# arturxe2/T-DEED

Hardware: AMD Instinct MI355X
Metric: clips/sec (L=100, 224^2, bf16) forward, per-frame logits (higher is better)
Workload: dtype bf16; 1 GPU; rny002_b8: rny002_gsf + ed_sgp_mixer n_layers=2 ks=7, L=100, 224x224, batch 8/GPU, inference forward, random-init weights; clips_per_gpu=8, parallelism=dp1 (clip-sharded, no collective), hip_graph=True, batches_in_flight=3, sub_batches_per_batch=1, dist_backend=none, dist_ranks=1, self_launched=False

## Files before the change

t-deed_amd/csrc/bneck.hip:

```cpp
#include "common.h"
#include "se_excite.h"

struct BneckP {
  const bf16_t* x; const bf16_t* G; int Fp;
  const bf16x8* w1f; const float* s1; const float* h1;
  const bf16x8* w2f; const float* s2; const float* h2;
  SeP se;
  const bf16x8* w3f; const float* s3; const float* h3;
  bf16_t* out; bf16_t* out2; int n2;
  int N, h, w, C;
  int w2_tap_major;
  long long* dbg;
  struct Gs {
    const bf16_t* x; int ldx;
    const float* gate; const float* ysum; const float* xsum;
    const float* cw1; const float* cb1; const float* cw2; const float* cb2;
    int T_len, F;
  } gs;
  struct Qt {
    const bf16x8* wqf;
    const float* bn;
    float* Q;
    int F;
  } qt;
// ... 154 lines not shown
#pragma unroll
      for (int b = 0; b < NLD; ++b) {
        const int i = i0 + b * BNK_THR;
        if (i < total) {
          int px, ck;
          dcpr.divmod(i, px, ck);
          ck += ck0;
          TD_LDS_CHECK(px * RS + ck * 16, 16, FPW * hw * RS);
          *reinterpret_cast<u32x4*>(At + px * RS + ck * 16) = v[b];
        }
      }
    };
    x_issue(tid);
    TD_ISSUE_FENCE();
    if (blend) {
      if (sfs < nfr && sc_ < gF) {
        const int f = f0 + sfs, t = f - dgt.div(f) * gT;
#pragma unroll
        for (int row = 0; row < 10; ++row) {
          const int t2 = t + (row >= 5 ? row - 5 : row) - 2;
          srow(1 + 12 * sfs + row)[sc_] = (t2 >= 0 && t2 < gT) ? sv[row] : 0.f;
        }
      }
      float* cwl = srow(1 + 12 * FPW);
      if (tid >= 256 && tid < 256 + 38) cwl[tid - 256] = cwv;
      __syncthreads();
      {
        const int fs = (FPW > 1 && tid >= p.Fp) ? 1 : 0, c = tid - fs * p.Fp;
        if (fs < nfr && c < p.Fp) {
          const int t = (f0 + fs) - dgt.div(f0 + fs) * gT;
          const int rb = 1 + 12 * fs;
          const float inv_hw = 1.0f / (float)hw;
          float wgt = 0.f;
          if (c < gF) {
            const int g = c >= gFh;
            const int cl = c - g * gFh;
            const float* cw = cwl + 18 * g;
            float a = cwl[36 + g];
#pragma unroll
            for (int dc = -1; dc <= 1; ++dc) {
              const int c2 = cl + dc;
              if (c2 < 0 || c2 >= gFh) continue;
              const int cc = g * gFh + c2;
#pragma unroll
              for (int dt = -1; dt <= 1; ++dt) {
                const int t2 = t + dt;
                if (t2 < 0 || t2 >= gT) continue;
                const float rm = (srow(rb + 5 + dt + 2)[cc] - srow(rb + dt + 2)[cc]) * inv_hw;
                const int r2 = dt + 2 + (g ? -1 : 1);
                const float ysh = srow(rb + r2)[cc] * inv_hw;
                a = fmaf(cw[(dc + 1) * 3 + (dt + 1)], ysh, a);
                a = fmaf(cw[9 + (dc + 1) * 3 + (dt + 1)], rm, a);
              }
            }
            wgt = sigmoidf_(a);
          }
          TD_LDS_CHECK((Bt - smem) + (rb + 11) * RS + c * 4, 4, (Zr - smem));
          srow(rb + 10)[c] = wgt;
          srow(rb + 11)[c] = 1.0f - wgt;
        }
      }
      __syncthreads();
      const IDiv dnpc(npc8);
#pragma unroll
      for (int j = 0; j < 3; ++j) {
        const int i = tid + j * BNK_THR;
        if (i < npix * npc8) {
          int px, ck;
          dnpc.divmod(i, px, ck);
          const int fs = (FPW > 1 && px >= hw) ? 1 : 0;
          const int t = (f0 + fs) - dgt.div(f0 + fs) * gT;
          const bool has_next = t < gT - 1, has_prev = t > 0;
          const float* fwl = srow(1 + 12 * fs + 10) + ck * 8;
          const float* oml = srow(1 + 12 * fs + 11) + ck * 8;
          const f32x4 w0 = *reinterpret_cast<const f32x4*>(fwl), w1 = *reinterpret_cast<const f32x4*>(fwl + 4);
          const f32x4 m0 = *reinterpret_cast<const f32x4*>(oml), m1 = *reinterpret_cast<const f32x4*>(oml + 4);
          const float gn_ = has_next ? bgn[j] : 0.f, gp_ = has_prev ? bgp[j] : 0.f;
          const bool lo_piece = ck * 8 < gFh;
          u32x4 o;
#pragma unroll
          for (int pr = 0; pr < 4; ++pr) {
            const int ci = ck * 8 + 2 * pr;
            const bool g = ci >= gFh;
            const unsigned xcw = bxc[j][pr], nbw = (g && lo_piece) ? bxp[j][pr] : bxn[j][pr];
            const f32x2 xv = {__builtin_bit_cast(float, xcw << 16), __builtin_bit_cast(float, xcw & 0xffff0000u)};
            const f32x2 nb = {__builtin_bit_cast(float, nbw << 16), __builtin_bit_cast(float, nbw & 0xffff0000u)};
            const float gate = g ? bga[j][1] : bga[j][0], gsh = g ? gp_ : gn_;
            const f32x2 gate2 = {gate, gate}, gsh2 = {gsh, gsh};
            const f32x2 wv = pr < 2 ? (f32x2){w0[2 * pr], w0[2 * pr + 1]} : (f32x2){w1[2 * pr - 4], w1[2 * pr - 3]};
            const f32x2 om = pr < 2 ? (f32x2){m0[2 * pr], m0[2 * pr + 1]} : (f32x2){m1[2 * pr - 4], m1[2 * pr - 3]};
            const f32x2 r = __builtin_elementwise_fma(-gate2, xv, xv);
            const f32x2 ysh = gsh2 * nb;
            const f32x2 t = r * om;
            const f32x2 ov = __builtin_elementwise_fma(ysh, wv, t);
            const bf16x2 ob = {(bf16_t)ov[0], (bf16_t)ov[1]};
            o[pr] = ci < gF ? __builtin_bit_cast(unsigned, ob) : xcw;
          }
          TD_LDS_CHECK(px * RS + ck * 16, 16, FPW * hw * RS);
          *reinterpret_cast<u32x4*>(At + px * RS + ck * 16) = o;
        }
      }
    }
    x_store(tid);
    for (int i0 = tid + BNK_THR * NLD; i0 < total; i0 += BNK_THR * NLD) {
      x_issue(i0);
      TD_ISSUE_FENCE();
      x_store(i0);
    }
    const int padp = (RS - C * 2) >> 4;
    for (int i = tid; i < 2 * FPW * hw * padp; i += BNK_THR) {
      const int r = i / padp, j = i - r * padp;
      *reinterpret_cast<u32x4*>(smem + r * RS + C * 2 + j * 16) = (u32x4){0u, 0u, 0u, 0u};
    }
    for (int i = tid; i < (RS + 64) >> 4; i += BNK_THR) *reinterpret_cast<u32x4*>(Zr + i * 16) = (u32x4){0u, 0u, 0u, 0u};
    if (tid < 4) *reinterpret_cast<u32x4*>(At + npix * RS + tid * 16) = (u32x4){0u, 0u, 0u, 0u};
#pragma unroll
    for (int j = 0; j < NBV; ++j) {
      const int i = tid + j * BNK_THR;
      if (i < 6 * CP) bnv[i] = (i - (i / CP) * CP) < C ? bv[j] : 0.f;
    }
  }
  __syncthreads();
  BN_STAMP(1);

  int prow[NPTM], srowA[NPTM];
#pragma unroll
  for (int pt = 0; pt < NPTM; ++pt) {
    const int px = pt * 16 + pl;
    prow[pt] = (px < npix ? px : 0) * RS;
    srowA[pt] = px < npix ? px * RS : (int)(Tr - At);
  }
  const int dAB = (int)(Bt - At);
  constexpr int HA = (NPTM + 1) / 2;
  auto contract = [&](const bf16x8 (&wc)[KS], const unsigned char* act, f32x4 (&acc)[NPTM]) {
#pragma unroll
    for (int pt = 0; pt < NPTM; ++pt) acc[pt] = (f32x4){0.f, 0.f, 0.f, 0.f};
    bf16x8 a[NPTM];
    const int kq = 16 * q;
#pragma unroll
    for (int pt = 0; pt < HA; ++pt) a[pt] = *reinterpret_cast<const bf16x8*>(act + prow[pt] + kq);
#pragma unroll
    for (int ks = 0; ks < KS; ++ks) {
      const int kb = 64 * ks + kq;
#pragma unroll
      for (int pt = HA; pt < NPTM; ++pt) a[pt] = *reinterpret_cast<const bf16x8*>(act + prow[pt] + kb);
#pragma unroll
      for (int pt = 0; pt < HA; ++pt) acc[pt] = __builtin_amdgcn_mfma_f32_16x16x32_bf16(wc[ks], a[pt], acc[pt], 0, 0, 0);
      __builtin_amdgcn_sched_barrier(0);
      if (ks + 1 < KS) {
#pragma unroll
        for (int pt = 0; pt < HA; ++pt) a[pt] = *reinterpret_cast<const bf16x8*>(act + prow[pt] + kb + 64);
      }
#pragma unroll
      for (int pt = HA; pt < NPTM; ++pt) acc[pt] = __builtin_amdgcn_mfma_f32_16x16x32_bf16(wc[ks], a[pt], acc[pt], 0, 0, 0);
      __builtin_amdgcn_sched_barrier(0);
    }
  };

  auto contract_half = [&](const bf16x8 (&wb)[KS], int ks0, const unsigned char* act, f32x4 (&acc0)[NPTM], f32x4 (&acc1)[NPTM]) {
    bf16x8 a[NPTM];
    const int kq = 16 * q;
#pragma unroll
    for (int pt = 0; pt < HA; ++pt) a[pt] = *reinterpret_cast<const bf16x8*>(act + prow[pt] + 64 * ks0 + kq);
#pragma unroll
    for (int k = 0; k < KH; ++k) {
      const int kb = 64 * (ks0 + k) + kq;
#pragma unroll
      for (int pt = HA; pt < NPTM; ++pt) a[pt] = *reinterpret_cast<const bf16x8*>(act + prow[pt] + kb);
#pragma unroll
      for (int pt = 0; pt < HA; ++pt) {
        acc0[pt] = __builtin_amdgcn_mfma_f32_16x16x32_bf16(wb[k], a[pt], acc0[pt], 0, 0, 0);
        acc1[pt] = __builtin_amdgcn_mfma_f32_16x16x32_bf16(wb[KH + k], a[pt], acc1[pt], 0, 0, 0);
      }
      __builtin_amdgcn_sched_barrier(0);
      if (k + 1 < KH) {
#pragma unroll
        for (int pt = 0; pt < HA; ++pt) a[pt] = *reinterpret_cast<const bf16x8*>(act + prow[pt] + kb + 64);
      }
#pragma unroll
      for (int pt = HA; pt < NPTM; ++pt) {
        acc0[pt] = __builtin_amdgcn_mfma_f32_16x16x32_bf16(wb[k], a[pt], acc0[pt], 0, 0, 0);
        acc1[pt] = __builtin_amdgcn_mfma_f32_16x16x32_bf16(wb[KH + k], a[pt], acc1[pt], 0, 0, 0);
      }
      __builtin_amdgcn_sched_barrier(0);
    }
  };
  auto contract_third = [&](const bf16x8 (&wb)[KS], int ks0, const unsigned char* act, f32x4 (&acc0)[NPTM], f32x4 (&acc1)[NPTM],
                            f32x4 (&acc2)[NPTM]) {
    bf16x8 a[NPTM];
    const int kq = 16 * q;
#pragma unroll
    for (int pt = 0; pt < HA; ++pt) a[pt] = *reinterpret_cast<const bf16x8*>(act + prow[pt] + 64 * ks0 + kq);
#pragma unroll
    for (int k = 0; k < KT; ++k) {
      const int kb = 64 * (ks0 + k) + kq;
#pragma unroll
      for (int pt = HA; pt < NPTM; ++pt) a[pt] = *reinterpret_cast<const bf16x8*>(act + prow[pt] + kb);
#pragma unroll
      for (int pt = 0; pt < HA; ++pt) {
        acc0[pt] = __builtin_amdgcn_mfma_f32_16x16x32_bf16(wb[k], a[pt], acc0[pt], 0, 0, 0);
        acc1[pt] = __builtin_amdgcn_mfma_f32_16x16x32_bf16(wb[KT + k], a[pt], acc1[pt], 0, 0, 0);
        acc2[pt] = __builtin_amdgcn_mfma_f32_16x16x32_bf16(wb[2 * KT + k], a[pt], acc2[pt], 0, 0, 0);
      }
      __builtin_amdgcn_sched_barrier(0);
      if (k + 1 < KT) {
#pragma unroll
        for (int pt = 0; pt < HA; ++pt) a[pt] = *reinterpret_cast<const bf16x8*>(act + prow[pt] + kb + 64);
      }
#pragma unroll
      for (int pt = HA; pt < NPTM; ++pt) {
        acc0[pt] = __builtin_amdgcn_mfma_f32_16x16x32_bf16(wb[k], a[pt], acc0[pt], 0, 0, 0);
        acc1[pt] = __builtin_amdgcn_mfma_f32_16x16x32_bf16(wb[KT + k], a[pt], acc1[pt], 0, 0, 0);
        acc2[pt] = __builtin_amdgcn_mfma_f32_16x16x32_bf16(wb[2 * KT + k], a[pt], acc2[pt], 0, 0, 0);
      }
      __builtin_amdgcn_sched_barrier(0);
    }
  };
  auto epi1 = [&](int T, const f32x4 (&acc)[NPTM]) {
    const int ch0 = T * 16 + 4 * q;
    const f32x4 sc = *reinterpret_cast<const f32x4*>(bnv + ch0), sh = *reinterpret_cast<const f32x4*>(bnv + CP + ch0);
#pragma unroll
    for (int pt = 0; pt < NPTM; ++pt) {
      bf16x4 o;
#pragma unroll
      for (int r = 0; r < 4; ++r) o[r] = (bf16_t)fmaxf(acc[pt][r] * sc[r] + sh[r], 0.f);
      unsigned char* dst = At + srowA[pt];
      TD_LDS_CHECK(((srowA[pt] < dAB ? dst + dAB : dst) + ch0 * 2) - smem, 8, (Tr + RS) - smem);
      *reinterpret_cast<bf16x4*>((srowA[pt] < dAB ? dst + dAB : dst) + ch0 * 2) = o;
    }
  };

  if constexpr (TRIPLE) {
    bf16x8 (&wn)[KS] = wn1;
    f32x4 acc0[NPTM], acc1[NPTM], acc2[NPTM];
#pragma unroll
    for (int pt = 0; pt < NPTM; ++pt) acc0[pt] = acc1[pt] = acc2[pt] = (f32x4){0.f, 0.f, 0.f, 0.f};
    contract_third(wc1, 0, At, acc0, acc1, acc2);
    load_block3(wc1, p.w1f, T3A, T3B, T3C, 2 * KT);
    contract_third(wn, KT, At, acc0, acc1, acc2);
    if (wv < NT) {
#pragma unroll
      for (int ks = 0; ks < 5; ++ks) wf2[ks] = p.w2f[((long)wv * 5 + ks) * 64 + lane];
    }
    contract_third(wc1, 2 * KT, At, acc0, acc1, acc2);
    epi1(T3A, acc0);
    epi1(T3B, acc1);
    if (t3c_ok) epi1(wv + 2 * BNK_NW, acc2);
  } else if constexpr (PAIR) {
    bf16x8 wn[KS];
    if (wv < NT) {
#pragma unroll
      for (int ks = 0; ks < 5; ++ks) wf2[ks] = p.w2f[((long)wv * 5 + ks) * 64 + lane];
    }
    const int TA = wv, TB = wv + BNK_NW, TC = wv + 2 * BNK_NW;
    load_block(wn, p.w1f, TA, TB, KH);
    f32x4 acc0[NPTM], acc1[NPTM];
#pragma unroll
    for (int pt = 0; pt < NPTM; ++pt) acc0[pt] = acc1[pt] = (f32x4){0.f, 0.f, 0.f, 0.f};
    contract_half(wc1, 0, At, acc0, acc1);
    if (TC < NT) {
#pragma unroll
      for (int ks = 0; ks < KS; ++ks) wc1[ks] = p.w1f[((long)TC * KS + ks) * 64 + lane];
    }
    contract_half(wn, KH, At, acc0, acc1);
    epi1(TA, acc0);
    epi1(TB, acc1);
    if (TC < NT) {
      contract(wc1, At, acc0);
      epi1(TC, acc0);
    }
  } else {
    bf16x8 (&wc)[KS] = wc1;
    bf16x8 wn[KS];
    if (wv < NT) {
#pragma unroll
      for (int ks = 0; ks < 5; ++ks) wf2[ks] = p.w2f[((long)wv * 5 + ks) * 64 + lane];
    }
    for (int T = wv; T < NT; T += BNK_NW) {
      if (T + BNK_NW < NT) {
#pragma unroll
        for (int ks = 0; ks < KS; ++ks) wn[ks] = p.w1f[((long)(T + BNK_NW) * KS + ks) * 64 + lane];
      }
      const int ch0 = T * 16 + 4 * q;
      const f32x4 sc = *reinterpret_cast<const f32x4*>(bnv + ch0), sh = *reinterpret_cast<const f32x4*>(bnv + CP + ch0);
      f32x4 acc[NPTM];
      contract(wc, At, acc);
#pragma unroll
      for (int pt = 0; pt < NPTM; ++pt) {
        bf16x4 o;
#pragma unroll
        for (int r = 0; r < 4; ++r) o[r] = (bf16_t)fmaxf(acc[pt][r] * sc[r] + sh[r], 0.f);
        unsigned char* dst = At + srowA[pt];
        TD_LDS_CHECK(((srowA[pt] < dAB ? dst + dAB : dst) + ch0 * 2) - smem, 8, (Tr + RS) - smem);
        *reinterpret_cast<bf16x4*>((srowA[pt] < dAB ? dst + dAB : dst) + ch0 * 2) = o;
      }
#pragma unroll
      for (int ks = 0; ks < KS; ++ks) wc[ks] = wn[ks];
    }
  }
  __syncthreads();
  BN_STAMP(2);

  bf16x8 sew1[KS];
  {
    const int NU = NT;
    int toff[NPTM][5];
    {
      const int zoff = (int)(Zr - Bt);
      int dyv[5], dxv[5], doff[5];
      bool sok[5];
#pragma unroll
      for (int ks = 0; ks < 5; ++ks) {
        const int sidx = 4 * ks + q;
        const int half = TAPM ? (sidx & 1) : (sidx >= 9 ? 1 : 0);
        const int tap = TAPM ? (sidx >> 1) : sidx - 9 * half;
        const int ty = (tap >= 3 ? 1 : 0) + (tap >= 6 ? 1 : 0);
        dyv[ks] = ty - 1;
        dxv[ks] = tap - 3 * ty - 1;
        sok[ks] = sidx < 18;
        doff[ks] = (dyv[ks] * p.w + dxv[ks]) * RS + half * 16;
      }
      const IDiv dhw(hw), dw(p.w);
#pragma unroll
      for (int pt = 0; pt < NPTM; ++pt) {
        const int px = min(pt * 16 + pl, npix - 1);
        int f, r, oy, ox;
        dhw.divmod(px, f, r);
        dw.divmod(r, oy, ox);
#pragma unroll
        for (int ks = 0; ks < 5; ++ks) {
          const bool ok = sok[ks] && (unsigned)(oy + dyv[ks]) < (unsigned)p.h && (unsigned)(ox + dxv[ks]) < (unsigned)p.w;
          toff[pt][ks] = ok ? px * RS + doff[ks] : zoff;
          TD_LDS_CHECK((Bt - smem) + toff[pt][ks] + (NT - 1) * 32, 16, lds_bytes);
        }
      }
    }
    constexpr int MAXU = KS <= 8 ? 2 : 3;
    bf16x8 wfx[MAXU - 1][5];
#pragma unroll
    for (int j = 1; j < MAXU; ++j) {
      const int U = min(wv + j * BNK_NW, NU - 1);
#pragma unroll
      for (int ks = 0; ks < 5; ++ks) wfx[j - 1][ks] = p.w2f[((long)U * 5 + ks) * 64 + lane];
    }
    BN_STAMP(8);
    auto unit = [&](int ju, const bf16x8 (&wfu)[5]) {
      const int U = wv + ju * BNK_NW;
      if (U >= NU) return;
      const int ch0 = U * 16 + 4 * q;
      const f32x4 sc = *reinterpret_cast<const f32x4*>(bnv + 2 * CP + ch0), sh = *reinterpret_cast<const f32x4*>(bnv + 3 * CP + ch0);
      float psum[FPW][4];
#pragma unroll
      for (int f = 0; f < FPW; ++f)
#pragma unroll
        for (int r = 0; r < 4; ++r) psum[f][r] = 0.f;
      f32x4 acc[NPTM];
#pragma unroll
      for (int pt = 0; pt < NPTM; ++pt) acc[pt] = (f32x4){0.f, 0.f, 0.f, 0.f};
      {
        bf16x8 yf[NPTM];
        const unsigned char* bu = Bt + U * 32;
#pragma unroll
        for (int pt = 0; pt < HA; ++pt) yf[pt] = *reinterpret_cast<const bf16x8*>(bu + toff[pt][0]);
#pragma unroll
        for (int ks = 0; ks < 5; ++ks) {
#pragma unroll
          for (int pt = HA; pt < NPTM; ++pt) yf[pt] = *reinterpret_cast<const bf16x8*>(bu + toff[pt][ks]);
#pragma unroll
          for (int pt = 0; pt < HA; ++pt) acc[pt] = __builtin_amdgcn_mfma_f32_16x16x32_bf16(wfu[ks], yf[pt], acc[pt], 0, 0, 0);
          __builtin_amdgcn_sched_barrier(0);
          if (ks + 1 < 5) {
#pragma unroll
            for (int pt = 0; pt < HA; ++pt) yf[pt] = *reinterpret_cast<const bf16x8*>(bu + toff[pt][ks + 1]);
          }
#pragma unroll
          for (int pt = HA; pt < NPTM; ++pt) acc[pt] = __builtin_amdgcn_mfma_f32_16x16x32_bf16(wfu[ks], yf[pt], acc[pt], 0, 0, 0);
          __builtin_amdgcn_sched_barrier(0);
        }
      }
#pragma unroll
      for (int pt = 0; pt < NPTM; ++pt) {
        const int px = pt * 16 + pl;
        const bool pok = px < npix;
        bf16x4 o;
#pragma unroll
        for (int r = 0; r < 4; ++r) o[r] = (bf16_t)fmaxf(acc[pt][r] * sc[r] + sh[r], 0.f);
        *reinterpret_cast<bf16x4*>(At + srowA[pt] + ch0 * 2) = o;
        const bool second = FPW > 1 && px >= hw;
#pragma unroll
        for (int r = 0; r < 4; ++r) {
          const float v = pok ? (float)o[r] : 0.f;
          if (FPW > 1) psum[FPW - 1][r] += second ? v : 0.f;
          psum[0][r] += second ? 0.f : v;
        }
      }
#pragma unroll
      for (int f = 0; f < FPW; ++f)
#pragma unroll
        for (int r = 0; r < 4; ++r) {
          const float v = bnk_row16_sum(psum[f][r]);
          if (pl == 0 && ch0 + r < C) pooled[f * C + ch0 + r] = v;
        }
      BN_STAMP(9 + ju);
    };
    auto se_prefetch = [&]() {
      const int KS1 = (C + 31) >> 5, RT = (p.se.R + 15) >> 4;
      const int tc = min(wv, RT - 1);
#pragma unroll
      for (int ks = 0; ks < KS; ++ks) sew1[ks] = p.se.w1f[((long)tc * KS1 + min(ks, KS1 - 1)) * 64 + lane];
    };
    unit(0, wf2);
    if constexpr (MAXU == 2) {
      se_prefetch();
      unit(1, wfx[0]);
    } else {
      unit(1, wfx[0]);
      se_prefetch();
      unit(2, wfx[MAXU - 2]);
    }
  }
  __syncthreads();
  BN_STAMP(3);

  bf16x8 wc3[KS];
  if constexpr (TRIPLE) {
    load_block3(wc3, p.w3f, T3A, T3B, T3C, 0);
  } else if constexpr (PAIR) {
    load_block(wc3, p.w3f, wv, wv + BNK_NW, 0);
  } else if (wv < NT) {
#pragma unroll
    for (int ks = 0; ks < KS; ++ks) wc3[ks] = p.w3f[((long)wv * KS + ks) * 64 + lane];
  }
  {
    SeP se = p.se;
    se.pooled = pooled; se.n_parts = 1; se.inv_cnt = 1.0f / (float)hw; se.C = C; se.gate_out = nullptr;
    se_excite_lds<KS, 3, true, BNK_NW, true>(se, 0, nfr, nfr - 1, gtab, C, Bt, p.dbg ? p.dbg + (long)blockIdx.x * 16 + 12 : nullptr,
                                             &sew1);
    const int cpr = C >> 3;
    const IDiv dcpr(cpr);
    for (int i = tid; i < npix * cpr; i += BNK_THR) {
      int px, ck;
      dcpr.divmod(i, px, ck);
      const float* g = gtab + ((FPW > 1 && px >= hw) ? C : 0) + ck * 8;
      bf16x8* ptr8 = reinterpret_cast<bf16x8*>(At + px * RS + ck * 16);
      bf16x8 v = *ptr8;
      const f32x4 g0 = *reinterpret_cast<const f32x4*>(g), g1 = *reinterpret_cast<const f32x4*>(g + 4);
#pragma unroll
      for (int e = 0; e < 4; ++e) {
        v[e] = (bf16_t)((float)v[e] * g0[e]);
        v[4 + e] = (bf16_t)((float)v[4 + e] * g1[e]);
      }
      *ptr8 = v;
    }
  }
  __syncthreads();
  BN_STAMP(4);

  const bool qtail = p.qt.Q != nullptr;
  const int qF = p.qt.F, nch = (qF + 7) >> 3, KSc = (nch + 3) >> 2, PSQ = (nch | 1) * 16;
  constexpr int QRSP = 224;
  unsigned char* qa = At;
  unsigned char* wl = qa + FPW * hw * PSQ;
  unsigned char* Pl = wl + 4 * KSc * 1024;
  u32x4 wr[2];
  f32x4 bs[3][2], bh[3][2];
  int ipx[3], ick[3];
  const IDiv dnch(qtail ? nch : 1), dw_(p.w), dhw_(hw);
  auto q_request = [&]() {
    if (!qtail) return;
#pragma unroll
    for (int b = 0; b < 2; ++b) wr[b] = reinterpret_cast<const u32x4*>(p.qt.wqf)[min(tid + b * BNK_THR, 4 * KSc * 64 - 1)];
  };
  auto q_request_bn = [&]() {
    if (!qtail) return;
#pragma unroll
    for (int j = 0; j < 3; ++j) {
      const int i = min(tid + j * BNK_THR, npix * nch - 1);
      dnch.divmod(i, ipx[j], ick[j]);
      const float* bq = p.qt.bn + ick[j] * 8;
      bs[j][0] = *reinterpret_cast<const f32x4*>(bq);
      bs[j][1] = *reinterpret_cast<const f32x4*>(bq + 4);
      bh[j][0] = *reinterpret_cast<const f32x4*>(bq + nch * 8);
      bh[j][1] = *reinterpret_cast<const f32x4*>(bq + nch * 8 + 4);
    }
  };
  auto load_res = [&](int T, bf16x4 (&rres)[NPTM]) {
    const int ch0 = T * 16 + 4 * q;
    const bool cok = ch0 < C;
#pragma unroll
    for (int pt = 0; pt < NPTM; ++pt) {
      const int px = pt * 16 + pl;
      rres[pt] = *reinterpret_cast<const bf16x4*>(xg + (long)((px < npix && cok) ? px : 0) * C + (cok ? ch0 : 0));
    }
  };
  auto epi3 = [&](int T, const f32x4 (&acc)[NPTM], const bf16x4 (&rres)[NPTM]) {
    const int ch0 = T * 16 + 4 * q;
    const f32x4 sc = *reinterpret_cast<const f32x4*>(bnv + 4 * CP + ch0), sh = *reinterpret_cast<const f32x4*>(bnv + 5 * CP + ch0);
#pragma unroll
    for (int pt = 0; pt < NPTM; ++pt) {
      bf16x4 o;
#pragma unroll
      for (int r = 0; r < 4; ++r) o[r] = (bf16_t)fmaxf(acc[pt][r] * sc[r] + sh[r] + (float)rres[pt][r], 0.f);
      unsigned char* dst = At + srowA[pt];
      *reinterpret_cast<bf16x4*>((srowA[pt] < dAB ? dst + dAB : dst) + ch0 * 2) = o;
    }
  };
  if constexpr (TRIPLE) {
    bf16x8 wn[KS];
    load_block3(wn, p.w3f, T3A, T3B, T3C, KT);
    f32x4 acc0[NPTM], acc1[NPTM], acc2[NPTM];
#pragma unroll
    for (int pt = 0; pt < NPTM; ++pt) acc0[pt] = acc1[pt] = acc2[pt] = (f32x4){0.f, 0.f, 0.f, 0.f};
    contract_third(wc3, 0, At, acc0, acc1, acc2);
    load_block3(wc3, p.w3f, T3A, T3B, T3C, 2 * KT);
    contract_third(wn, KT, At, acc0, acc1, acc2);
    bf16x4 rA[NPTM], rB[NPTM], rC[NPTM];
    load_res(T3A, rA);
    load_res(T3B, rB);
    load_res(T3C, rC);
    contract_third(wc3, 2 * KT, At, acc0, acc1, acc2);
    q_request();
    epi3(T3A, acc0, rA);
    epi3(T3B, acc1, rB);
    if (t3c_ok) epi3(wv + 2 * BNK_NW, acc2, rC);
  } else if constexpr (PAIR) {
    bf16x8 wn[KS];
    const int TA = wv, TB = wv + BNK_NW, TC = wv + 2 * BNK_NW;
    load_block(wn, p.w3f, TA, TB, KH);
    bf16x4 rA[NPTM], rB[NPTM];
    load_res(TA, rA);
    f32x4 acc0[NPTM], acc1[NPTM];
#pragma unroll
    for (int pt = 0; pt < NPTM; ++pt) acc0[pt] = acc1[pt] = (f32x4){0.f, 0.f, 0.f, 0.f};
    contract_half(wc3, 0, At, acc0, acc1);
    load_res(TB, rB);
    if (TC < NT) {
#pragma unroll
      for (int ks = 0; ks < KS; ++ks) wc3[ks] = p.w3f[((long)TC * KS + ks) * 64 + lane];
    }
    contract_half(wn, KH, At, acc0, acc1);
    if (!(TC < NT)) q_request();
    epi3(TA, acc0, rA);
    if (TC < NT) load_res(TC, rA);
    epi3(TB, acc1, rB);
    if (TC < NT) {
      contract(wc3, At, acc0);
      q_request();
      epi3(TC, acc0, rA);
    }
  } else {
    bf16x8 (&wc)[KS] = wc3;
    bf16x8 wn[KS];
    for (int T = wv; T < NT; T += BNK_NW) {
      if (T + BNK_NW < NT) {
#pragma unroll
        for (int ks = 0; ks < KS; ++ks) wn[ks] = p.w3f[((long)(T + BNK_NW) * KS + ks) * 64 + lane];
      }
      const int ch0 = T * 16 + 4 * q;
      const bool cok = ch0 < C;
      const f32x4 sc = *reinterpret_cast<const f32x4*>(bnv + 4 * CP + ch0), sh = *reinterpret_cast<const f32x4*>(bnv + 5 * CP + ch0);
      bf16x4 rres[NPTM];
#pragma unroll
      for (int pt = 0; pt < NPTM; ++pt) {
        const int px = pt * 16 + pl;
        rres[pt] = *reinterpret_cast<const bf16x4*>(xg + (long)((px < npix && cok) ? px : 0) * C + (cok ? ch0 : 0));
      }
      f32x4 acc[NPTM];
      contract(wc, At, acc);
#pragma unroll
      for (int pt = 0; pt < NPTM; ++pt) {
        bf16x4 o;
#pragma unroll
        for (int r = 0; r < 4; ++r) o[r] = (bf16_t)fmaxf(acc[pt][r] * sc[r] + sh[r] + (float)rres[pt][r], 0.f);
        unsigned char* dst = At + srowA[pt];
        *reinterpret_cast<bf16x4*>((srowA[pt] < dAB ? dst + dAB : dst) + ch0 * 2) = o;
      }
#pragma unroll
      for (int ks = 0; ks < KS; ++ks) wc[ks] = wn[ks];
    }
    q_request();
  }
  q_request_bn();
  __syncthreads();
  BN_STAMP(5);
  if (qtail) {
#pragma unroll
    for (int j = 0; j < 3; ++j) {
      if (tid + j * BNK_THR < npix * nch) {
        const bf16x8 v = *reinterpret_cast<const bf16x8*>(Bt + ipx[j] * RS + ick[j] * 16);
        bf16x8 o;
#pragma unroll
        for (int e = 0; e < 4; ++e) {
          o[e] = (bf16_t)fmaxf(fmaf((float)v[e], bs[j][0][e], bh[j][0][e]), 0.f);
          o[4 + e] = (bf16_t)fmaxf(fmaf((float)v[4 + e], bs[j][1][e], bh[j][1][e]), 0.f);
        }
        TD_LDS_CHECK(ipx[j] * PSQ + ick[j] * 16, 16, wl - smem);
        *reinterpret_cast<bf16x8*>(qa + ipx[j] * PSQ + ick[j] * 16) = o;
      }
    }
#pragma unroll
    for (int b = 0; b < 2; ++b)
      if (tid + b * BNK_THR < 4 * KSc * 64) {
        TD_LDS_CHECK((wl - smem) + (tid + b * BNK_THR) * 16, 16, Pl - smem);
        *reinterpret_cast<u32x4*>(wl + (tid + b * BNK_THR) * 16) = wr[b];
      }
    __syncthreads();
    BN_STAMP(8);
    constexpr int KSCM = (KS + 3) / 4;
    for (int pt = wv; pt * 16 < npix; pt += BNK_NW) {
      const int row = min(pt * 16 + pl, npix - 1);
      f32x4 acc[4];
#pragma unroll
      for (int rt = 0; rt < 4; ++rt) acc[rt] = (f32x4){0.f, 0.f, 0.f, 0.f};
#pragma unroll
      for (int ks = 0; ks < KSCM; ++ks) {
        if (ks < KSc) {
          const int chunk = 4 * ks + q;
          const bf16x8 av = *reinterpret_cast<const bf16x8*>(qa + row * PSQ + (chunk < nch ? chunk : 0) * 16);
#pragma unroll
          for (int rt = 0; rt < 4; ++rt)
            acc[rt] = __builtin_amdgcn_mfma_f32_16x16x32_bf16(*reinterpret_cast<const bf16x8*>(wl + ((rt * KSc + ks) * 64 + lane) * 16),
                                                              av, acc[rt], 0, 0, 0);
        }
      }
      if (pt * 16 + pl < npix) {
#pragma unroll
        for (int rt = 0; rt < 4; ++rt)
          if (rt * 16 + 4 * q < 56) {
            TD_LDS_CHECK((Pl - smem) + row * QRSP + (rt * 16 + 4 * q) * 4, 16, Bt - smem);
            *reinterpret_cast<f32x4*>(Pl + row * QRSP + (rt * 16 + 4 * q) * 4) = acc[rt];
          }
      }
    }
    __syncthreads();
    BN_STAMP(9);
    {
      const IDiv d6(6);
      for (int i = tid; i < npix * 6; i += BNK_THR) {
        int px, jg, fr, pix, py, pxx;
        d6.divmod(i, px, jg);
        dhw_.divmod(px, fr, pix);
        dw_.divmod(pix, py, pxx);
        float sum = 0.f;
#pragma unroll
        for (int tap = 0; tap < 9; ++tap) {
          const int dy = tap / 3 - 1, dx = tap % 3 - 1;
          const bool ok = (unsigned)(py + dy) < (unsigned)p.h && (unsigned)(pxx + dx) < (unsigned)p.w;
          const float v = *reinterpret_cast<const float*>(Pl + (ok ? px + dy * p.w + dx : px) * QRSP + (tap * 6 + jg) * 4);
          sum += ok ? v : 0.f;
        }
        p.qt.Q[((long)f0 * hw + px) * 6 + jg] = sum;
      }
    }
    BN_STAMP(7);
  }
  {
    const int cpr = C >> 3;
    const IDiv dcpr(cpr);
    bf16_t* og = p.out + (long)f0 * hw * C;
    for (int i = tid; i < npix * cpr; i += BNK_THR) {
      int px, ck;
      dcpr.divmod(i, px, ck);
      const u32x4 v = *reinterpret_cast<const u32x4*>(Bt + px * RS + ck * 16);
      *reinterpret_cast<u32x4*>(og + (long)px * C + ck * 8) = v;
      if (p.out2 && ck * 8 < p.n2) *reinterpret_cast<u32x4*>(p.out2 + ((long)f0 * hw + px) * p.n2 + ck * 8) = v;
    }
  }
  BN_STAMP(6);
}

static int bneck_fpw(int hw) { return hw <= 64 ? 2 : 1; }

static long long* g_bneck_dbg = nullptr;
extern "C" int tdeed_bneck_set_debug(void* buf) { g_bneck_dbg = (long long*)buf; return TDEED_OK; }

extern "C" int tdeed_bneck_fits(int h, int w, int C, int R) {
  const int hw = h * w, KS = (C + 31) / 32, fpw = bneck_fpw(hw);
  if (h < 3 || w < 3 || C % 8 != 0 || R < 1 || R > 96 || C > 384) return 0;
  if (!(KS == 5 || KS == 12)) return 0;
  if ((C + 15) / 16 > 3 * BNK_NW) return 0;
  if ((fpw * hw + 15) / 16 > (KS == 12 ? 7 : (fpw == 2 ? 8 : 13))) return 0;
  if ((size_t)se_excite_scratch_bytes(C, R) > (size_t)fpw * hw * bneck_rs(C)) return 0;
  return bneck_smem(fpw, hw, C) <= 160 * 1024 ? 1 : 0;
}

static int bneck_launch(BneckP& p, hipStream_t st) {
  const int h = p.h, w = p.w, C = p.C, N = p.N;
  p.dbg = g_bneck_dbg;
  const int hw = h * w, fpw = bneck_fpw(hw), KS = (C + 31) / 32;
  const size_t smem = bneck_smem(fpw, hw, C);
  static TdDevOnce attr_set;
  if (!attr_set.get()) {
    hipError_t e = hipSuccess;
#define BNK_ATTR(...) if (e == hipSuccess) e = hipFuncSetAttribute((const void*)bneck_kernel<__VA_ARGS__>, hipFuncAttributeMaxDynamicSharedMemorySize, 160 * 1024)
#define BNK_ATTR4(...) BNK_ATTR(__VA_ARGS__, true, true); BNK_ATTR(__VA_ARGS__, true, false); BNK_ATTR(__VA_ARGS__, false, true); \
                       BNK_ATTR(__VA_ARGS__, false, false)
    BNK_ATTR4(12, 2, 7); BNK_ATTR4(5, 1, 13); BNK_ATTR4(5, 2, 8); BNK_ATTR4(12, 1, 7);
#undef BNK_ATTR4
#undef BNK_ATTR
    if (e != hipSuccess) { tdeed_set_error("bneck: hipFuncSetAttribute: %s", hipGetErrorString(e)); return TDEED_ERR_RUNTIME; }
    attr_set.set();
  }
  const int grid = (N + fpw - 1) / fpw;
  const bool tm = p.w2_tap_major != 0;
  const bool bl = p.gs.gate != nullptr;
#define BNK_GO1(...) hipLaunchKernelGGL((bneck_kernel<__VA_ARGS__>), dim3(grid), dim3(BNK_THR), smem, st, p)
#define BNK_GO(...) do { if (tm && bl) BNK_GO1(__VA_ARGS__, true, true); else if (tm) BNK_GO1(__VA_ARGS__, true, false); \
                         else if (bl) BNK_GO1(__VA_ARGS__, false, true); else BNK_GO1(__VA_ARGS__, false, false); } while (0)
  if (KS == 12 && fpw == 2) BNK_GO(12, 2, 7);
  else if (KS == 5 && fpw == 1) BNK_GO(5, 1, 13);
  else if (KS == 5 && fpw == 2) BNK_GO(5, 2, 8);
  else if (KS == 12 && fpw == 1) BNK_GO(12, 1, 7);
  else { tdeed_set_error("bneck: KS=%d with %d frames per workgroup", KS, fpw); return TDEED_ERR_ARG; }
#undef BNK_GO
#undef BNK_GO1
  TD_LAUNCH_CHECK("bneck");
  return TDEED_OK;
}

static int bneck_fill(BneckP& p, const void* x, int N, int h, int w, int C, const void* w1f, const float* s1, const float* h1,
                      const void* w2f, const float* s2, const float* h2, const void* se_w1f, const float* se_b1,
                      const void* se_w2f, const float* se_b2, int R, const void* w3f, const float* s3, const float* h3, void* out,
                      void* out2, int n2, int w2_tap_major) {
  TD_CHECK(x && w1f && s1 && h1 && w2f && s2 && h2 && se_w1f && se_b1 && se_w2f && se_b2 && w3f && s3 && h3 && out,
           "bneck: null pointer");
  TD_CHECK(N > 0 && tdeed_bneck_fits(h, w, C, R), "bneck: geometry h=%d w=%d C=%d R=%d unsupported", h, w, C, R);
  TD_CHECK(!out2 || (n2 % 8 == 0 && n2 > 0 && n2 <= C), "bneck: bad second output width %d", n2);
  p = BneckP{};
  p.x = (const bf16_t*)x;
  p.w1f = (const bf16x8*)w1f; p.s1 = s1; p.h1 = h1;
  p.w2f = (const bf16x8*)w2f; p.s2 = s2; p.h2 = h2;
  p.se = SeP{};
  p.se.R = R; p.se.w1f = (const bf16x8*)se_w1f; p.se.b1 = se_b1; p.se.w2f = (const bf16x8*)se_w2f; p.se.b2 = se_b2;
  p.w3f = (const bf16x8*)w3f; p.s3 = s3; p.h3 = h3;
  p.out = (bf16_t*)out; p.out2 = (bf16_t*)out2; p.n2 = out2 ? n2 : 0;
  p.N = N; p.h = h; p.w = w; p.C = C;
  p.w2_tap_major = w2_tap_major ? 1 : 0;
  return TDEED_OK;
}

extern "C" int tdeed_bneck_qtail_fits(int h, int w, int C, int F) {
  if (F <= 0 || F % 4 != 0 || 2 * F > C) return 0;
  const int hw = h * w, fpw = bneck_fpw(hw), nch = (F + 7) / 8, KSc = (nch + 3) / 4, PSQ = (nch | 1) * 16;
  if (nch > (C + 31) / 32 || 4 * KSc * 64 > 2 * BNK_THR || fpw * hw * nch > 3 * BNK_THR) return 0;
  return (size_t)fpw * hw * (PSQ + 224) + (size_t)4 * KSc * 1024 <= (size_t)fpw * hw * bneck_rs(C) ? 1 : 0;
}

extern "C" int tdeed_bneck_fwd(const void* x, const void* G, int Fp, int N, int h, int w, int C, const void* w1f,
                               const float* s1, const float* h1, const void* w2f, const float* s2, const float* h2,
                               const void* se_w1f, const float* se_b1, const void* se_w2f, const float* se_b2, int R,
                               const void* w3f, const float* s3, const float* h3, void* out, void* out2, int n2,
                               int w2_tap_major, void* stream) {
  BneckP p;
  const int rc = bneck_fill(p, x, N, h, w, C, w1f, s1, h1, w2f, s2, h2, se_w1f, se_b1, se_w2f, se_b2, R, w3f, s3, h3, out, out2, n2,
                            w2_tap_major);
  if (rc != TDEED_OK) return rc;
  TD_CHECK(!G || (Fp % 8 == 0 && Fp > 0 && Fp <= C), "bneck: bad splice width %d", Fp);
  p.G = (const bf16_t*)G; p.Fp = G ? Fp : 0;
  return bneck_launch(p, (hipStream_t)stream);
}

extern "C" int tdeed_bneck_gs_fwd(const void* x, const void* gx, int ldx, const float* gate, const float* ysum, const float* xsum,
                                  const float* cw1, const float* cb1, const float* cw2, const float* cb2, int T, int F, int Fp,
                                  int N, int h, int w, int C, const void* w1f, const float* s1, const float* h1, const void* w2f,
                                  const float* s2, const float* h2, const void* se_w1f, const float* se_b1, const void* se_w2f,
                                  const float* se_b2, int R, const void* w3f, const float* s3, const float* h3, void* out,
                                  void* out2, int n2, int w2_tap_major, const void* q_wqf, const float* q_bn, int q_F, float* Q,
                                  void* stream) {
  BneckP p;
  const int rc = bneck_fill(p, x, N, h, w, C, w1f, s1, h1, w2f, s2, h2, se_w1f, se_b1, se_w2f, se_b2, R, w3f, s3, h3, out, out2, n2,
                            w2_tap_major);
  if (rc != TDEED_OK) return rc;
  if (Q) {
    TD_CHECK(q_wqf && q_bn, "bneck_gs: tap maps asked for without fragments / BatchNorm table");
    TD_CHECK(tdeed_bneck_qtail_fits(h, w, C, q_F), "bneck_gs: the tap-map tail does not fit (h=%d w=%d C=%d F=%d)", h, w, C, q_F);
    p.qt.wqf = (const bf16x8*)q_wqf; p.qt.bn = q_bn; p.qt.Q = Q; p.qt.F = q_F;
  }
  TD_CHECK(gx && gate && ysum && xsum && cw1 && cb1 && cw2 && cb2, "bneck_gs: null pointer");
  TD_CHECK(F % 4 == 0 && F > 0 && Fp % 8 == 0 && Fp >= F && Fp < F + 8 && 2 * Fp <= C && ldx >= Fp && ldx % 8 == 0,
           "bneck_gs: bad fold F=%d Fp=%d ldx=%d C=%d", F, Fp, ldx, C);
  TD_CHECK(T > 0 && N % T == 0 && N < (1 << 22), "bneck_gs: %d frames are not whole clips of %d", N, T);
  const int hw = h * w, fpw = bneck_fpw(hw);
  TD_CHECK(hw >= 14 && fpw * hw * (Fp / 8) <= 3 * BNK_THR && fpw * Fp <= BNK_THR,
           "bneck_gs: a %d x %d map with a %d-channel slice does not fit the blend's scratch / piece slots", h, w, Fp);
  p.Fp = Fp;
  p.gs.x = (const bf16_t*)gx; p.gs.ldx = ldx; p.gs.gate = gate; p.gs.ysum = ysum; p.gs.xsum = xsum;
  p.gs.cw1 = cw1; p.gs.cb1 = cb1; p.gs.cw2 = cw2; p.gs.cb2 = cb2; p.gs.T_len = T; p.gs.F = F;
  return bneck_launch(p, (hipStream_t)stream);
}
```

t-deed_amd/csrc/se_excite.h:

```cpp
#pragma once
#include "common.h"

struct SeP {
  const float* pooled;
  int n_parts;
  float inv_cnt;
  int C, R;
  const bf16x8* w1f;
  const float* b1;
  const bf16x8* w2f;
  const float* b2;
  float* gate_out;
};

__host__ __device__ inline int se_excite_scratch_bytes(int C, int R) {
  const int KS1 = (C + 31) >> 5, KS2 = (R + 31) >> 5;
  return 2 * 16 * (KS1 * 32 + 8) * 2 + 2 * 16 * (KS2 * 32 + 8) * 2;
}

#define SE_LDS_BARRIER()                                               \
  do {                                                                 \
    __builtin_amdgcn_fence(__ATOMIC_RELEASE, "workgroup", "local");    \
    __builtin_amdgcn_s_barrier();                                      \
    __builtin_amdgcn_fence(__ATOMIC_ACQUIRE, "workgroup", "local");    \
  } while (0)
template <int KS1M, int KS2M, bool EARLY = true, int NW = 4, bool PRE = false>
__device__ __forceinline__ void se_excite_lds(const SeP& se, long f_first, int nf, long f_last, float* gtab, int ldg,
                                              unsigned char* scratch, long long* stamps = nullptr,
                                              const bf16x8 (*w1pre)[KS1M] = nullptr) {
  const int C = se.C, R = se.R;
  const int KS1 = (C + 31) >> 5, RT = (R + 15) >> 4, CT = (C + 15) >> 4, KS2 = (R + 31) >> 5;
  const int PS1 = KS1 * 32 + 8, PS2 = KS2 * 32 + 8;
  bf16_t* Phi = reinterpret_cast<bf16_t*>(scratch);
  bf16_t* Plo = Phi + 16 * PS1;
  bf16_t* Hhi = Plo + 16 * PS1;
  bf16_t* Hlo = Hhi + 16 * PS2;
  const int tid = threadIdx.x, lane = tid & 63, wv = tid >> 6, pl = lane & 15, q = lane >> 4;
  bf16x8 w1r[KS1M];
  if constexpr (PRE) {
#pragma unroll
    for (int ks = 0; ks < KS1M; ++ks) w1r[ks] = (*w1pre)[ks];
  } else if constexpr (EARLY) {
    const int tc = min(wv, RT - 1);
#pragma unroll
    for (int ks = 0; ks < KS1M; ++ks) w1r[ks] = se.w1f[((long)tc * KS1 + min(ks, KS1 - 1)) * 64 + lane];
  }
  constexpr int MAXT2 = (24 + NW - 1) / NW;
  bf16x8 w2r[EARLY ? MAXT2 : 1][KS2M];
  if constexpr (EARLY) {
#pragma unroll
    for (int j = 0; j < MAXT2; ++j) {
      const int tc = min(wv + j * NW, CT - 1);
#pragma unroll
      for (int ks = 0; ks < KS2M; ++ks) w2r[j][ks] = se.w2f[((long)tc * KS2 + min(ks, KS2 - 1)) * 64 + lane];
    }
  }
  constexpr int MAXT1 = (6 + NW - 1) / NW;
  float b1v[MAXT1][4], b2v[MAXT2][4];
#pragma unroll
  for (int j = 0; j < MAXT1; ++j)
#pragma unroll
    for (int e = 0; e < 4; ++e) b1v[j][e] = se.b1[min((wv + j * NW) * 16 + 4 * q + e, R - 1)];
#pragma unroll
  for (int j = 0; j < MAXT2; ++j)
#pragma unroll
    for (int e = 0; e < 4; ++e) b2v[j][e] = se.b2[min((wv + j * NW) * 16 + 4 * q + e, C - 1)];
  const int c4n = KS1 * 8;
  for (int i = tid; i < 16 * c4n; i += NW * 64) {
    const int f = i / c4n, c = (i - f * c4n) * 4;
    f32x4 acc = {0.f, 0.f, 0.f, 0.f};
    if (f < nf && c < C) {
      const float* src = se.pooled + (min(f_first + f, f_last) * se.n_parts) * (long)C + c;
      for (int p = 0; p < se.n_parts; ++p) {
        const f32x4 v = *reinterpret_cast<const f32x4*>(src + (long)p * C);
        acc[0] += v[0]; acc[1] += v[1]; acc[2] += v[2]; acc[3] += v[3];
      }
    }
    bf16x4 hi, lo;
#pragma unroll
    for (int e = 0; e < 4; ++e) {
      const float m = acc[e] * se.inv_cnt;
      hi[e] = (bf16_t)m;
      lo[e] = (bf16_t)(m - (float)hi[e]);
    }
    TD_LDS_CHECK((f * PS1 + c) * 2, 8, 16 * PS1 * 2);
    *reinterpret_cast<bf16x4*>(Phi + f * PS1 + c) = hi;
    *reinterpret_cast<bf16x4*>(Plo + f * PS1 + c) = lo;
  }
  for (int i = tid; i < 2 * 16 * PS2 / 8; i += NW * 64) reinterpret_cast<u32x4*>(Hhi)[i] = (u32x4){0u, 0u, 0u, 0u};
  SE_LDS_BARRIER();
  if (stamps && tid == 0) stamps[0] = clock64();
#pragma unroll
  for (int j1 = 0; j1 < MAXT1; ++j1) {
    const int tile = wv + j1 * NW;
    if (tile >= RT) break;
    if (!(EARLY || PRE) || tile != wv) {
#pragma unroll
      for (int ks = 0; ks < KS1M; ++ks) w1r[ks] = se.w1f[((long)tile * KS1 + min(ks, KS1 - 1)) * 64 + lane];
    }
    f32x4 acc = {0.f, 0.f, 0.f, 0.f};
#pragma unroll
    for (int ks = 0; ks < KS1M; ++ks)
      if (ks < KS1) {
        const bf16x8 bh = *reinterpret_cast<const bf16x8*>(Phi + pl * PS1 + ks * 32 + q * 8);
        const bf16x8 bl = *reinterpret_cast<const bf16x8*>(Plo + pl * PS1 + ks * 32 + q * 8);
        acc = __builtin_amdgcn_mfma_f32_16x16x32_bf16(w1r[ks], bh, acc, 0, 0, 0);
        acc = __builtin_amdgcn_mfma_f32_16x16x32_bf16(w1r[ks], bl, acc, 0, 0, 0);
      }
#pragma unroll
    for (int e = 0; e < 4; ++e) {
      const int r = tile * 16 + 4 * q + e;
      const float hv = r < R ? fmaxf(acc[e] + b1v[j1][e], 0.f) : 0.f;
      const bf16_t hi = (bf16_t)hv;
      Hhi[pl * PS2 + r] = hi;
      Hlo[pl * PS2 + r] = (bf16_t)(hv - (float)hi);
    }
  }
  SE_LDS_BARRIER();
  if (stamps && tid == 0) stamps[1] = clock64();
#pragma unroll
  for (int j = 0; j < MAXT2; ++j) {
    const int tile = wv + j * NW;
    if (tile >= CT) break;
    bf16x8 wt[KS2M];
#pragma unroll
    for (int ks = 0; ks < KS2M; ++ks) {
      if constexpr (EARLY) wt[ks] = w2r[j][ks];
      else wt[ks] = se.w2f[((long)tile * KS2 + min(ks, KS2 - 1)) * 64 + lane];
    }
    f32x4 acc = {0.f, 0.f, 0.f, 0.f};
#pragma unroll
    for (int ks = 0; ks < KS2M; ++ks)
      if (ks < KS2) {
        const bf16x8 bh = *reinterpret_cast<const bf16x8*>(Hhi + pl * PS2 + ks * 32 + q * 8);
        const bf16x8 bl = *reinterpret_cast<const bf16x8*>(Hlo + pl * PS2 + ks * 32 + q * 8);
        acc = __builtin_amdgcn_mfma_f32_16x16x32_bf16(wt[ks], bh, acc, 0, 0, 0);
        acc = __builtin_amdgcn_mfma_f32_16x16x32_bf16(wt[ks], bl, acc, 0, 0, 0);
      }
    const int c0 = tile * 16 + 4 * q;
    if (c0 < C && pl < nf) {
      f32x4 g;
#pragma unroll
      for (int e = 0; e < 4; ++e) g[e] = sigmoid_fast_(acc[e] + b2v[j][e]);
      TD_DEV_ASSERT(pl < 16 && c0 + 4 <= ldg);
      *reinterpret_cast<f32x4*>(gtab + pl * ldg + c0) = g;
      if (se.gate_out && f_first + pl <= f_last) *reinterpret_cast<f32x4*>(se.gate_out + (f_first + pl) * (long)C + c0) = g;
    }
  }
  SE_LDS_BARRIER();
  if (stamps && tid == 0) stamps[2] = clock64();
}
```

Measured before the change: 5999 clips/s.

## Issue conv3 and SE fc2 weight loads behind last depthwise unit MFMAs

Moves the global loads for the third 1x1 conv weights and the SE excitation fc2 weights and biases earlier, into the final grouped-conv unit between its MFMA loop and epilogue. Waves with no unit still run these loads. The second conv3 weight block is also loaded before the SE gating loop. The goal is to hide global-load latency behind MFMA work and barriers, at the cost of more live VGPRs, which may lower occupancy or cause spills.

```diff
diff --git a/t-deed_amd/csrc/bneck.hip b/t-deed_amd/csrc/bneck.hip
--- a/t-deed_amd/csrc/bneck.hip
+++ b/t-deed_amd/csrc/bneck.hip
@@ -480,6 +480,8 @@
   BN_STAMP(2);
 
   bf16x8 sew1[KS];
+  bf16x8 wc3[KS];
+  SePre2<3, BNK_NW> sepre;
   {
     const int NU = NT;
     int toff[NPTM][5];
@@ -522,20 +524,14 @@
       for (int ks = 0; ks < 5; ++ks) wfx[j - 1][ks] = p.w2f[((long)U * 5 + ks) * 64 + lane];
     }
     BN_STAMP(8);
-    auto unit = [&](int ju, const bf16x8 (&wfu)[5]) {
+    auto unit = [&](int ju, const bf16x8 (&wfu)[5], auto&& behind) {
       const int U = wv + ju * BNK_NW;
-      if (U >= NU) return;
+      const bool mine = U < NU;
       const int ch0 = U * 16 + 4 * q;
-      const f32x4 sc = *reinterpret_cast<const f32x4*>(bnv + 2 * CP + ch0), sh = *reinterpret_cast<const f32x4*>(bnv + 3 * CP + ch0);
-      float psum[FPW][4];
-#pragma unroll
-      for (int f = 0; f < FPW; ++f)
-#pragma unroll
-        for (int r = 0; r < 4; ++r) psum[f][r] = 0.f;
       f32x4 acc[NPTM];
 #pragma unroll
       for (int pt = 0; pt < NPTM; ++pt) acc[pt] = (f32x4){0.f, 0.f, 0.f, 0.f};
-      {
+      if (mine) {
         bf16x8 yf[NPTM];
         const unsigned char* bu = Bt + U * 32;
 #pragma unroll
@@ -556,6 +552,15 @@
           __builtin_amdgcn_sched_barrier(0);
         }
       }
+      behind();
+      __builtin_amdgcn_sched_barrier(0);
+      if (!mine) return;
+      const f32x4 sc = *reinterpret_cast<const f32x4*>(bnv + 2 * CP + ch0), sh = *reinterpret_cast<const f32x4*>(bnv + 3 * CP + ch0);
+      float psum[FPW][4];
+#pragma unroll
+      for (int f = 0; f < FPW; ++f)
+#pragma unroll
+        for (int r = 0; r < 4; ++r) psum[f][r] = 0.f;
 #pragma unroll
       for (int pt = 0; pt < NPTM; ++pt) {
         const int px = pt * 16 + pl;
@@ -587,33 +592,50 @@
 #pragma unroll
       for (int ks = 0; ks < KS; ++ks) sew1[ks] = p.se.w1f[((long)tc * KS1 + min(ks, KS1 - 1)) * 64 + lane];
     };
-    unit(0, wf2);
+    auto c3_prefetch = [&]() {
+      if constexpr (TRIPLE) {
+        load_block3(wc3, p.w3f, T3A, T3B, T3C, 0);
+      } else if constexpr (PAIR) {
+        load_block(wc3, p.w3f, wv, wv + BNK_NW, 0);
+      } else {
+        const int tc = min(wv, NT - 1);
+#pragma unroll
+        for (int ks = 0; ks < KS; ++ks) wc3[ks] = p.w3f[((long)tc * KS + ks) * 64 + lane];
+      }
+    };
+    auto nothing = [] {};
+    auto last_requests = [&]() {
+      c3_prefetch();
+      se_excite_request2(p.se, C, p.se.R, sepre);
+    };
+    unit(0, wf2, nothing);
     if constexpr (MAXU == 2) {
       se_prefetch();
-      unit(1, wfx[0]);
+      unit(1, wfx[0], last_requests);
     } else {
-      unit(1, wfx[0]);
+      unit(1, wfx[0], nothing);
       se_prefetch();
-      unit(2, wfx[MAXU - 2]);
+      unit(2, wfx[MAXU - 2], last_requests);
     }
   }
   __syncthreads();
   BN_STAMP(3);
 
-  bf16x8 wc3[KS];
-  if constexpr (TRIPLE) {
-    load_block3(wc3, p.w3f, T3A, T3B, T3C, 0);
-  } else if constexpr (PAIR) {
-    load_block(wc3, p.w3f, wv, wv + BNK_NW, 0);
-  } else if (wv < NT) {
-#pragma unroll
-    for (int ks = 0; ks < KS; ++ks) wc3[ks] = p.w3f[((long)wv * KS + ks) * 64 + lane];
-  }
+  bf16x8 wn3[KS];
   {
     SeP se = p.se;
     se.pooled = pooled; se.n_parts = 1; se.inv_cnt = 1.0f / (float)hw; se.C = C; se.gate_out = nullptr;
-    se_excite_lds<KS, 3, true, BNK_NW, true>(se, 0, nfr, nfr - 1, gtab, C, Bt, p.dbg ? p.dbg + (long)blockIdx.x * 16 + 12 : nullptr,
-                                             &sew1);
+    se_excite_lds<KS, 3, true, BNK_NW, true, true>(se, 0, nfr, nfr - 1, gtab, C, Bt,
+                                                   p.dbg ? p.dbg + (long)blockIdx.x * 16 + 12 : nullptr, &sew1, &sepre);
+    if constexpr (TRIPLE) {
+      load_block3(wn3, p.w3f, T3A, T3B, T3C, KT);
+    } else if constexpr (PAIR) {
+      load_block(wn3, p.w3f, wv, wv + BNK_NW, KH);
+    } else {
+      const int tn = min(wv + BNK_NW, NT - 1);
+#pragma unroll
+      for (int ks = 0; ks < KS; ++ks) wn3[ks] = p.w3f[((long)tn * KS + ks) * 64 + lane];
+    }
     const int cpr = C >> 3;
     const IDiv dcpr(cpr);
     for (int i = tid; i < npix * cpr; i += BNK_THR) {
@@ -672,7 +694,8 @@
     }
   };
   auto epi3 = [&](int T, const f32x4 (&acc)[NPTM], const bf16x4 (&rres)[NPTM]) {
-    const int ch0 = T * 16 + 4 * q;
+    int ch0 = T * 16 + 4 * q;
+    asm volatile("" : "+v"(ch0));
     const f32x4 sc = *reinterpret_cast<const f32x4*>(bnv + 4 * CP + ch0), sh = *reinterpret_cast<const f32x4*>(bnv + 5 * CP + ch0);
 #pragma unroll
     for (int pt = 0; pt < NPTM; ++pt) {
@@ -684,8 +707,7 @@
     }
   };
   if constexpr (TRIPLE) {
-    bf16x8 wn[KS];
-    load_block3(wn, p.w3f, T3A, T3B, T3C, KT);
+    bf16x8 (&wn)[KS] = wn3;
     f32x4 acc0[NPTM], acc1[NPTM], acc2[NPTM];
 #pragma unroll
     for (int pt = 0; pt < NPTM; ++pt) acc0[pt] = acc1[pt] = acc2[pt] = (f32x4){0.f, 0.f, 0.f, 0.f};
@@ -702,9 +724,8 @@
     epi3(T3B, acc1, rB);
     if (t3c_ok) epi3(wv + 2 * BNK_NW, acc2, rC);
   } else if constexpr (PAIR) {
-    bf16x8 wn[KS];
+    bf16x8 (&wn)[KS] = wn3;
     const int TA = wv, TB = wv + BNK_NW, TC = wv + 2 * BNK_NW;
-    load_block(wn, p.w3f, TA, TB, KH);
     bf16x4 rA[NPTM], rB[NPTM];
     load_res(TA, rA);
     f32x4 acc0[NPTM], acc1[NPTM];
@@ -728,11 +749,14 @@
     }
   } else {
     bf16x8 (&wc)[KS] = wc3;
-    bf16x8 wn[KS];
+    bf16x8 (&wn)[KS] = wn3;
+#pragma nounroll
     for (int T = wv; T < NT; T += BNK_NW) {
-      if (T + BNK_NW < NT) {
-#pragma unroll
-        for (int ks = 0; ks < KS; ++ks) wn[ks] = p.w3f[((long)(T + BNK_NW) * KS + ks) * 64 + lane];
+      if constexpr (KS > 8) {
+        if (T != wv && T + BNK_NW < NT) {
+#pragma unroll
+          for (int ks = 0; ks < KS; ++ks) wn[ks] = p.w3f[((long)(T + BNK_NW) * KS + ks) * 64 + lane];
+        }
       }
       const int ch0 = T * 16 + 4 * q;
       const bool cok = ch0 < C;
diff --git a/t-deed_amd/csrc/se_excite.h b/t-deed_amd/csrc/se_excite.h
--- a/t-deed_amd/csrc/se_excite.h
+++ b/t-deed_amd/csrc/se_excite.h
@@ -24,10 +24,36 @@
     __builtin_amdgcn_s_barrier();                                      \
     __builtin_amdgcn_fence(__ATOMIC_ACQUIRE, "workgroup", "local");    \
   } while (0)
-template <int KS1M, int KS2M, bool EARLY = true, int NW = 4, bool PRE = false>
+template <int KS2M, int NW>
+struct SePre2 {
+  static constexpr int MAXT1 = (6 + NW - 1) / NW, MAXT2 = (24 + NW - 1) / NW;
+  bf16x8 w2r[MAXT2][KS2M];
+  float b1v[MAXT1][4], b2v[MAXT2][4];
+};
+template <int KS2M, int NW>
+__device__ __forceinline__ void se_excite_request2(const SeP& se, int C, int R, SePre2<KS2M, NW>& d) {
+  const int CT = (C + 15) >> 4, KS2 = (R + 31) >> 5;
+  const int lane = threadIdx.x & 63, wv = threadIdx.x >> 6, q = lane >> 4;
+#pragma unroll
+  for (int j = 0; j < SePre2<KS2M, NW>::MAXT1; ++j)
+#pragma unroll
+    for (int e = 0; e < 4; ++e) d.b1v[j][e] = se.b1[min((wv + j * NW) * 16 + 4 * q + e, R - 1)];
+#pragma unroll
+  for (int j = 0; j < SePre2<KS2M, NW>::MAXT2; ++j) {
+    const int tc = min(wv + j * NW, CT - 1);
+#pragma unroll
+    for (int ks = 0; ks < KS2M; ++ks) d.w2r[j][ks] = se.w2f[((long)tc * KS2 + min(ks, KS2 - 1)) * 64 + lane];
+  }
+#pragma unroll
+  for (int j = 0; j < SePre2<KS2M, NW>::MAXT2; ++j)
+#pragma unroll
+    for (int e = 0; e < 4; ++e) d.b2v[j][e] = se.b2[min((wv + j * NW) * 16 + 4 * q + e, C - 1)];
+}
+template <int KS1M, int KS2M, bool EARLY = true, int NW = 4, bool PRE = false, bool PRE2 = false>
 __device__ __forceinline__ void se_excite_lds(const SeP& se, long f_first, int nf, long f_last, float* gtab, int ldg,
                                               unsigned char* scratch, long long* stamps = nullptr,
-                                              const bf16x8 (*w1pre)[KS1M] = nullptr) {
+                                              const bf16x8 (*w1pre)[KS1M] = nullptr, const SePre2<KS2M, NW>* pre2 = nullptr) {
+  static_assert(!PRE2 || EARLY, "pre-requested fc2 fragments take the place of the EARLY ones");
   const int C = se.C, R = se.R;
   const int KS1 = (C + 31) >> 5, RT = (R + 15) >> 4, CT = (C + 15) >> 4, KS2 = (R + 31) >> 5;
   const int PS1 = KS1 * 32 + 8, PS2 = KS2 * 32 + 8;
@@ -47,7 +73,12 @@
   }
   constexpr int MAXT2 = (24 + NW - 1) / NW;
   bf16x8 w2r[EARLY ? MAXT2 : 1][KS2M];
-  if constexpr (EARLY) {
+  if constexpr (PRE2) {
+#pragma unroll
+    for (int j = 0; j < MAXT2; ++j)
+#pragma unroll
+      for (int ks = 0; ks < KS2M; ++ks) w2r[j][ks] = pre2->w2r[j][ks];
+  } else if constexpr (EARLY) {
 #pragma unroll
     for (int j = 0; j < MAXT2; ++j) {
       const int tc = min(wv + j * NW, CT - 1);
@@ -60,11 +91,11 @@
 #pragma unroll
   for (int j = 0; j < MAXT1; ++j)
 #pragma unroll
-    for (int e = 0; e < 4; ++e) b1v[j][e] = se.b1[min((wv + j * NW) * 16 + 4 * q + e, R - 1)];
+    for (int e = 0; e < 4; ++e) b1v[j][e] = PRE2 ? pre2->b1v[j][e] : se.b1[min((wv + j * NW) * 16 + 4 * q + e, R - 1)];
 #pragma unroll
   for (int j = 0; j < MAXT2; ++j)
 #pragma unroll
-    for (int e = 0; e < 4; ++e) b2v[j][e] = se.b2[min((wv + j * NW) * 16 + 4 * q + e, C - 1)];
+    for (int e = 0; e < 4; ++e) b2v[j][e] = PRE2 ? pre2->b2v[j][e] : se.b2[min((wv + j * NW) * 16 + 4 * q + e, C - 1)];
   const int c4n = KS1 * 8;
   for (int i = tid; i < 16 * c4n; i += NW * 64) {
     const int f = i / c4n, c = (i - f * c4n) * 4;
```

Result: no change. 6018 clips/s (median of 2 runs) (+0.3%).
